# RoboticsDesignLab/jitterbug

Measured on AMD Instinct MI355X. Metric: env steps/s at N_envs=4096, move_from_origin, higher is better.
Workload: dtype f32

## Files before the change

jitterbug_amd/csrc/jb_lane.hpp:

```cpp
#pragma once
#include <cmath>
#include <cstdint>
#include <type_traits>
#if !defined(__HIPCC__)
#include <atomic>
#include <thread>
#endif

#if defined(__HIPCC__)
#include <hip/hip_runtime.h>
#define JB_HD __host__ __device__ __forceinline__
#define JB_D __device__ __forceinline__
#else
#define JB_HD inline
#define JB_D inline
#endif

namespace jb {

#if defined(__HIPCC__)
JB_D float dpp_quad_xor1(float x) {
    return __builtin_bit_cast(float, __builtin_amdgcn_update_dpp(0, __builtin_bit_cast(int, x), 0xB1, 0xF, 0xF, false));
}
JB_D float dpp_quad_xor2(float x) {
    return __builtin_bit_cast(float, __builtin_amdgcn_update_dpp(0, __builtin_bit_cast(int, x), 0x4E, 0xF, 0xF, false));
}
JB_D float quad_sum(float x) {
    x += dpp_quad_xor1(x);
    x += dpp_quad_xor2(x);
    return x;
}
JB_D unsigned quad_sum_u(unsigned x) {
    x += (unsigned)__builtin_amdgcn_update_dpp(0, (int)x, 0xB1, 0xF, 0xF, false);
    x += (unsigned)__builtin_amdgcn_update_dpp(0, (int)x, 0x4E, 0xF, 0xF, false);
    return x;
}
JB_D bool any_lane(bool m) { return __builtin_amdgcn_ballot_w64(m) != 0ull; }
JB_D unsigned xor_sum_bits(unsigned u, int off, bool sym2, bool is_float) {
    auto add = [&](unsigned a, unsigned b) { return is_float ? __builtin_bit_cast(unsigned, __builtin_bit_cast(float, a) + __builtin_bit_cast(float, b)) : a + b; };
    if (off == 32) { auto r = __builtin_amdgcn_permlane32_swap(u, u, false, false); return add(r[0], r[1]); }
    if (off == 16) { auto r = __builtin_amdgcn_permlane16_swap(u, u, false, false); return add(r[0], r[1]); }
    if (off == 8) return add(u, (unsigned)__builtin_amdgcn_update_dpp(0, (int)u, 0x128, 0xF, 0xF, false));
    if (off == 4 && sym2) return add(u, (unsigned)__builtin_amdgcn_update_dpp(0, (int)u, 0x124, 0xF, 0xF, false));
    return add(u, (unsigned)__shfl_xor((int)u, off, 64));
}
JB_D float row_transpose_sum(float v0, float v1, float v2, float v3) {
    auto f = [](unsigned u) { return __builtin_bit_cast(float, u); };
    auto b = [](float x) { return __builtin_bit_cast(unsigned, x); };
    auto r02 = __builtin_amdgcn_permlane32_swap(b(v0), b(v2), false, false);
    auto r13 = __builtin_amdgcn_permlane32_swap(b(v1), b(v3), false, false);
    float s02 = f(r02[0]) + f(r02[1]), s13 = f(r13[0]) + f(r13[1]);
    auto r = __builtin_amdgcn_permlane16_swap(b(s02), b(s13), false, false);
    return f(r[0]) + f(r[1]);
}
JB_D unsigned xor_get_bits(unsigned u, int off) {
    if (off == 32) { auto r = __builtin_amdgcn_permlane32_swap(u, u, false, false); return r[1]; }
    if (off == 16) { auto r = __builtin_amdgcn_permlane16_swap(u, u, false, false); return r[1]; }
    if (off == 8) return (unsigned)__builtin_amdgcn_update_dpp(0, (int)u, 0x128, 0xF, 0xF, false);
    return (unsigned)__shfl_xor((int)u, off, 64);
}
JB_D unsigned xor_get_any_u(unsigned u, int off) {
    if (off == 32) { auto r = __builtin_amdgcn_permlane32_swap(u, u, false, false); return r[0] ^ r[1] ^ u; }
    if (off == 16) { auto r = __builtin_amdgcn_permlane16_swap(u, u, false, false); return r[0] ^ r[1] ^ u; }
    return xor_get_bits(u, off);
}
JB_D float xor_get(float x, int off) { return __builtin_bit_cast(float, xor_get_bits(__builtin_bit_cast(unsigned, x), off)); }
JB_D unsigned xor_get_u(unsigned x, int off) { return xor_get_bits(x, off); }
template <int J> JB_D float quad_bcast(float x) { return __builtin_bit_cast(float, __builtin_amdgcn_update_dpp(0, __builtin_bit_cast(int, x), J * 0x55, 0xF, 0xF, false)); }
JB_D float xor_sum(float x, int off, bool sym2) { return __builtin_bit_cast(float, xor_sum_bits(__builtin_bit_cast(unsigned, x), off, sym2, true)); }
JB_D unsigned xor_sum_u(unsigned x, int off, bool sym2) { return xor_sum_bits(x, off, sym2, false); }
JB_D unsigned wave_bcast_u(unsigned x) { return (unsigned)__builtin_amdgcn_readfirstlane((int)x); }
JB_D void wave_sync() {
    __builtin_amdgcn_fence(__ATOMIC_RELEASE, "wavefront");
    __builtin_amdgcn_wave_barrier();
    __builtin_amdgcn_fence(__ATOMIC_ACQUIRE, "wavefront");
}
template <int K> JB_D float quad_rot(float x) {
    constexpr int ctrl = K == 1 ? 0x39 : K == 2 ? 0x4E : 0x93;
    return __builtin_bit_cast(float, __builtin_amdgcn_update_dpp(0, __builtin_bit_cast(int, x), ctrl, 0xF, 0xF, false));
}
template <int K> JB_D unsigned quad_rot_u(unsigned x) {
    constexpr int ctrl = K == 1 ? 0x39 : K == 2 ? 0x4E : 0x93;
    return (unsigned)__builtin_amdgcn_update_dpp(0, (int)x, ctrl, 0xF, 0xF, false);
}
template <int J> JB_D unsigned quad_bcast_u(unsigned x) { return (unsigned)__builtin_amdgcn_update_dpp(0, (int)x, J * 0x55, 0xF, 0xF, false); }
JB_D unsigned quad_lane_id(const float*) { return threadIdx.x & 3u; }
JB_D float ld_leg(const float* p, int stride, unsigned idx, unsigned src, unsigned me) { return p[(int)(idx * (unsigned)stride) + (int)src - (int)me]; }
JB_D void st_leg(float* p, int stride, unsigned idx, unsigned src, unsigned me, float v, bool on) { if (on) p[(int)(idx * (unsigned)stride) + (int)src - (int)me] = v; }
JB_D float quad_pick(float x, unsigned src) {
    const int xi = __builtin_bit_cast(int, x);
    const float x0 = __builtin_bit_cast(float, __builtin_amdgcn_update_dpp(0, xi, 0x00, 0xF, 0xF, false)), x1 = __builtin_bit_cast(float, __builtin_amdgcn_update_dpp(0, xi, 0x55, 0xF, 0xF, false));
    const float x2 = __builtin_bit_cast(float, __builtin_amdgcn_update_dpp(0, xi, 0xAA, 0xF, 0xF, false)), x3 = __builtin_bit_cast(float, __builtin_amdgcn_update_dpp(0, xi, 0xFF, 0xF, 0xF, false));
    const float lo = (src & 1u) ? x1 : x0, hi = (src & 1u) ? x3 : x2;
    return (src & 2u) ? hi : lo;
}
#endif

JB_HD float sel(bool m, float a, float b) { return m ? a : b; }
JB_HD double sel(bool m, double a, double b) { return m ? a : b; }
JB_HD unsigned selu(bool m, unsigned a, unsigned b) { return m ? a : b; }
JB_HD bool lt(float a, float b) { return a < b; }
JB_HD bool lt(double a, double b) { return a < b; }
JB_HD bool gt(float a, float b) { return a > b; }
JB_HD bool gt(double a, double b) { return a > b; }
JB_HD bool mand(bool a, bool b) { return a && b; }
JB_HD bool mor(bool a, bool b) { return a || b; }
JB_HD bool mnot(bool a) { return !a; }
JB_HD unsigned mbit(bool a) { return a ? 1u : 0u; }
JB_HD unsigned popc_u(unsigned a) { return (unsigned)__builtin_popcount(a); }
JB_HD unsigned xor_u(unsigned a, unsigned b) { return a ^ b; }
JB_HD bool eq_u(unsigned a, unsigned b) { return a == b; }
JB_HD bool lt_u(unsigned a, unsigned b) { return a < b; }
JB_HD unsigned or_u(unsigned a, unsigned b) { return a | b; }
JB_HD unsigned and_u(unsigned a, unsigned b) { return a & b; }
JB_HD unsigned sub_u(unsigned a, unsigned b) { return a - b; }
JB_HD unsigned shl_u(unsigned a, unsigned s) { return a << s; }
JB_HD unsigned ctz_u(unsigned a) { return a ? (unsigned)__builtin_ctz(a) : 0u; }
JB_HD unsigned clear_low_u(unsigned a) { return a & (a - 1u); }
JB_HD float utov(unsigned a, const float*) { return (float)a; }
JB_HD double utov(unsigned a, const double*) { return (double)a; }
JB_HD void flip_decode(unsigned diff0, unsigned diff1, unsigned rec0, unsigned rec1, unsigned live, unsigned& entry, bool& is_flip, bool& plus, bool& tan2, bool& on) {
    const bool w1 = diff0 == 0u;
    const unsigned diff = w1 ? diff1 : diff0, rec = w1 ? rec1 : rec0;
// ... 101 lines not shown
inline void wave_sync() { if (g_host_wave) g_host_wave->barrier(); }
template <typename T> inline Quad<T> host_exchange(const Quad<T>& x, int partner) {
    HostWave* w = g_host_wave;
    for (int i = 0; i < 4; i++) w->mbox[g_host_grp][0][i] = (double)x.v[i];
    w->barrier();
    Quad<T> r;
    for (int i = 0; i < 4; i++) r.v[i] = (T)w->mbox[partner][0][i];
    w->barrier();
    return r;
}
template <typename T> inline Quad<T> row_transpose_sum(const Quad<T>& v0, const Quad<T>& v1, const Quad<T>& v2, const Quad<T>& v3) {
    HostWave* w = g_host_wave;
    if (!w) return v0;
    const Quad<T>* v[4] = {&v0, &v1, &v2, &v3};
    for (int k = 0; k < 4; k++) for (int i = 0; i < 4; i++) w->mbox[g_host_grp][k][i] = (double)v[k]->v[i];
    w->barrier();
    Quad<T> r;
    const int g = g_host_grp;
    for (int i = 0; i < 4; i++) r.v[i] = ((T)w->mbox[0][g][i] + (T)w->mbox[2][g][i]) + ((T)w->mbox[1][g][i] + (T)w->mbox[3][g][i]);
    w->barrier();
    return r;
}
template <typename T> inline Quad<T> xor_sum(const Quad<T>& x, int off, bool) {
    if (!g_host_wave) return x;
    return x + host_exchange(x, g_host_grp ^ (off / g_host_wave->gstride));
}
inline UQuad xor_sum_u(const UQuad& x, int off, bool) {
    HostWave* w = g_host_wave;
    if (!w) return x;
    for (int i = 0; i < 4; i++) w->umbox[g_host_grp][i] = x.v[i];
    w->barrier();
    UQuad r;
    const int partner = g_host_grp ^ (off / w->gstride);
    for (int i = 0; i < 4; i++) r.v[i] = x.v[i] + w->umbox[partner][i];
    w->barrier();
    return r;
}
template <typename T> inline Quad<T> xor_get(const Quad<T>& x, int off) {
    if (!g_host_wave) return x;
    return host_exchange(x, g_host_grp ^ (off / g_host_wave->gstride));
}
inline UQuad xor_get_u(const UQuad& x, int off) {
    HostWave* w = g_host_wave;
    if (!w) return x;
    for (int i = 0; i < 4; i++) w->umbox[g_host_grp][i] = x.v[i];
    w->barrier();
    UQuad r;
    const int partner = g_host_grp ^ (off / w->gstride);
    for (int i = 0; i < 4; i++) r.v[i] = w->umbox[partner][i];
    w->barrier();
    return r;
}
inline UQuad xor_get_any_u(const UQuad& x, int off) { return xor_get_u(x, off); }
template <int J, typename T> inline Quad<T> quad_bcast(const Quad<T>& x) { return Quad<T>(x.v[J]); }
inline unsigned wave_bcast_u(unsigned x) {
    HostWave* w = g_host_wave;
    if (!w) return x;
    w->umbox[g_host_grp][0] = x;
    w->barrier();
    const unsigned r = w->umbox[0][0];
    w->barrier();
    return r;
}
inline bool any_lane(bool m) { return m; }
inline float quad_sum(float x) { return x; }
inline double quad_sum(double x) { return x; }
template <typename T> inline Quad<T> sel(const Mask4& m, const Quad<T>& a, const Quad<T>& b) { Quad<T> r; for (int i = 0; i < 4; i++) r.v[i] = m.v[i] ? a.v[i] : b.v[i]; return r; }
inline UQuad selu(const Mask4& m, const UQuad& a, const UQuad& b) { UQuad r; for (int i = 0; i < 4; i++) r.v[i] = m.v[i] ? a.v[i] : b.v[i]; return r; }
template <typename T> inline Mask4 lt(const Quad<T>& a, const Quad<T>& b) { Mask4 r; for (int i = 0; i < 4; i++) r.v[i] = a.v[i] < b.v[i]; return r; }
template <typename T> inline Mask4 gt(const Quad<T>& a, const Quad<T>& b) { Mask4 r; for (int i = 0; i < 4; i++) r.v[i] = a.v[i] > b.v[i]; return r; }
inline Mask4 mand(const Mask4& a, const Mask4& b) { Mask4 r; for (int i = 0; i < 4; i++) r.v[i] = a.v[i] && b.v[i]; return r; }
inline Mask4 mor(const Mask4& a, const Mask4& b) { Mask4 r; for (int i = 0; i < 4; i++) r.v[i] = a.v[i] || b.v[i]; return r; }
inline Mask4 mnot(const Mask4& a) { Mask4 r; for (int i = 0; i < 4; i++) r.v[i] = !a.v[i]; return r; }
inline UQuad mbit(const Mask4& a) { UQuad r; for (int i = 0; i < 4; i++) r.v[i] = a.v[i] ? 1u : 0u; return r; }
inline UQuad popc_u(const UQuad& a) { UQuad r; for (int i = 0; i < 4; i++) r.v[i] = (uint32_t)__builtin_popcount(a.v[i]); return r; }
inline UQuad xor_u(const UQuad& a, const UQuad& b) { UQuad r; for (int i = 0; i < 4; i++) r.v[i] = a.v[i] ^ b.v[i]; return r; }
inline Mask4 lt_u(const UQuad& a, uint32_t b) { Mask4 r; for (int i = 0; i < 4; i++) r.v[i] = a.v[i] < b; return r; }
inline UQuad or_u(const UQuad& a, const UQuad& b) { UQuad r; for (int i = 0; i < 4; i++) r.v[i] = a.v[i] | b.v[i]; return r; }
inline UQuad and_u(const UQuad& a, const UQuad& b) { UQuad r; for (int i = 0; i < 4; i++) r.v[i] = a.v[i] & b.v[i]; return r; }
inline UQuad and_u(const UQuad& a, uint32_t b) { UQuad r; for (int i = 0; i < 4; i++) r.v[i] = a.v[i] & b; return r; }
inline UQuad sub_u(const UQuad& a, const UQuad& b) { UQuad r; for (int i = 0; i < 4; i++) r.v[i] = a.v[i] - b.v[i]; return r; }
inline UQuad shl_u(const UQuad& a, const UQuad& s) { UQuad r; for (int i = 0; i < 4; i++) r.v[i] = a.v[i] << s.v[i]; return r; }
inline UQuad ctz_u(const UQuad& a) { UQuad r; for (int i = 0; i < 4; i++) r.v[i] = a.v[i] ? (uint32_t)__builtin_ctz(a.v[i]) : 0u; return r; }
inline UQuad clear_low_u(const UQuad& a) { UQuad r; for (int i = 0; i < 4; i++) r.v[i] = a.v[i] & (a.v[i] - 1u); return r; }
inline Mask4 lt_u(const UQuad& a, const UQuad& b) { Mask4 r; for (int i = 0; i < 4; i++) r.v[i] = a.v[i] < b.v[i]; return r; }
inline Mask4 eq_u(const UQuad& a, uint32_t b) { Mask4 r; for (int i = 0; i < 4; i++) r.v[i] = a.v[i] == b; return r; }
template <typename T> inline Quad<T> utov(const UQuad& a, const Quad<T>*) { Quad<T> r; for (int i = 0; i < 4; i++) r.v[i] = (T)a.v[i]; return r; }
template <int K, typename T> inline Quad<T> quad_rot(const Quad<T>& x) { Quad<T> r; for (int i = 0; i < 4; i++) r.v[i] = x.v[(i + K) & 3]; return r; }
template <int K> inline UQuad quad_rot_u(const UQuad& x) { UQuad r; for (int i = 0; i < 4; i++) r.v[i] = x.v[(i + K) & 3]; return r; }
template <int J> inline UQuad quad_bcast_u(const UQuad& x) { return UQuad{{x.v[J], x.v[J], x.v[J], x.v[J]}}; }
template <typename T> inline UQuad quad_lane_id(const Quad<T>*) { return UQuad{{0u, 1u, 2u, 3u}}; }
template <typename T> inline void st_leg(Quad<T>* p, int stride, const UQuad& idx, const UQuad& src, const UQuad&, const Quad<T>& v, const Mask4& on) { for (int i = 0; i < 4; i++) if (on.v[i]) p[idx.v[i] * stride].v[src.v[i]] = v.v[i]; }
template <typename T> inline Quad<T> quad_pick(const Quad<T>& x, const UQuad& src) { Quad<T> r; for (int i = 0; i < 4; i++) r.v[i] = x.v[src.v[i]]; return r; }
template <typename T> inline Quad<T> ld_leg(const Quad<T>* p, int stride, const UQuad& idx, const UQuad& src, const UQuad&) { Quad<T> r; for (int i = 0; i < 4; i++) r.v[i] = p[idx.v[i] * stride].v[src.v[i]]; return r; }
inline Mask4 eq_u(const UQuad& a, const UQuad& b) { Mask4 r; for (int i = 0; i < 4; i++) r.v[i] = a.v[i] == b.v[i]; return r; }
inline void flip_decode(const UQuad& diff0, const UQuad& diff1, const UQuad& rec0, const UQuad& rec1, unsigned live, UQuad& entry, Mask4& is_flip, Mask4& plus, Mask4& tan2, Mask4& on) {
    for (int i = 0; i < 4; i++) flip_decode(diff0.v[i], diff1.v[i], rec0.v[i], rec1.v[i], live, entry.v[i], is_flip.v[i], plus.v[i], tan2.v[i], on.v[i]);
}
template <typename T> inline Quad<T> ld_gather(const Quad<T>* p, int stride, const UQuad& idx) { Quad<T> r; for (int i = 0; i < 4; i++) r.v[i] = p[idx.v[i] * stride].v[i]; return r; }
inline Mask4 neq_u(const UQuad& a, const UQuad& b) { Mask4 r; for (int i = 0; i < 4; i++) r.v[i] = a.v[i] != b.v[i]; return r; }
inline UQuad operator*(const UQuad& a, uint32_t b) { UQuad r; for (int i = 0; i < 4; i++) r.v[i] = a.v[i] * b; return r; }
inline UQuad operator+(const UQuad& a, const UQuad& b) { UQuad r; for (int i = 0; i < 4; i++) r.v[i] = a.v[i] + b.v[i]; return r; }
inline UQuad operator+(const UQuad& a, uint32_t b) { UQuad r; for (int i = 0; i < 4; i++) r.v[i] = a.v[i] + b; return r; }
#define JB_QUN(name, fn) template <typename T> inline Quad<T> name(const Quad<T>& a) { Quad<T> r; for (int i = 0; i < 4; i++) r.v[i] = fn(a.v[i]); return r; }
template <typename T> inline Quad<T> vmul_rn(const Quad<T>& a, const Quad<T>& b) { Quad<T> r; for (int i = 0; i < 4; i++) r.v[i] = vmul_rn(a.v[i], b.v[i]); return r; }
template <typename T> inline Quad<T> vadd_rn(const Quad<T>& a, const Quad<T>& b) { Quad<T> r; for (int i = 0; i < 4; i++) r.v[i] = vadd_rn(a.v[i], b.v[i]); return r; }
// ... 55 lines not shown
```

jitterbug_amd/csrc/jb_sim.hpp:

```cpp
#pragma once
#include <type_traits>
#if !defined(__HIPCC__)
#include <cstdio>
#endif

#include "jb_lane.hpp"

#if defined(__HIPCC__) && defined(__HIP_DEVICE_COMPILE__)
#define JB_SCHED_FENCE() __builtin_amdgcn_sched_barrier(0)
#define JB_ASM_MARK(txt) asm volatile("; " txt)
#else
#define JB_ASM_MARK(txt) ((void)0)
#define JB_NO_DEVICE_PROF 1
#define JB_SCHED_FENCE() ((void)0)
#endif

#if defined(JB_WAVE_STATS) && !defined(JB_NO_DEVICE_PROF)
#define JB_PROF_T0() unsigned long long _pt = __builtin_amdgcn_s_memtime()
#define JB_PROF_ADD(o, i) do { unsigned long long _n = __builtin_amdgcn_s_memtime(); if ((o).prof) (o).prof[i] += _n - _pt; _pt = _n; } while (0)
#else
#define JB_PROF_T0() ((void)0)
#define JB_PROF_ADD(o, i) ((void)0)
#endif

// ... 242 lines not shown
    V fail;
#ifdef JB_WAVE_STATS
    V st_fast, st_checks;
    V st_xtra, st_sweeps, st_contact, st_slots;
#endif
};

constexpr int NSLOT = 30, SLOT_THREAD = 28, SLOT_MASS = 29;
constexpr int ROW_F = 13;
constexpr int ROW_K = JB_ROW_K;
enum SC : int {
    SC_DD = 0 ,
    SC_Y = 24 ,
    SC_ST = SC_Y + 9 ,
    SC_OWN = SC_ST + 6 ,
    SC_ROWS = SC_OWN + 1 ,
    SC_VAR = SC_ROWS + ROW_K * ROW_F ,
    SC_RED = SC_VAR ,
    SC_OVC = SC_RED + 56 ,
    SC_PD = SC_OVC + 4 * (NSLOT - ROW_K) ,
    SC_PD2 = SC_PD + 12 ,
    SC_ZERO = SC_PD2 + 9 ,
    SC_COUNT = SC_ZERO + 56,
    SC_SYS = SC_VAR , SC_FAC = SC_SYS + 41 , SC_LSTATE = SC_FAC + 43 ,
    SC_COUNT_LEAN = SC_LSTATE + 36,
    SC_CX_LEAN = SC_COUNT_LEAN , SC_PD_LEAN = SC_CX_LEAN + 2 , SC_COUNT_LEAN_PAIR = SC_PD_LEAN + 12
};
template <typename V> struct LaneScratch {
    V* p;
    int stride;
    int grp, ngrp, gstride;
    V* ovc;
    int ovc_stride;
    int pd;
    int pd2;
    bool aux_lane = false;
    bool red_lds;
    JB_HD V ld(int i) const { return p[i * stride]; }
    JB_HD void st(int i, const V& v) const { p[i * stride] = v; }
    JB_HD V ldv(const typename lane_traits<V>::uint& i) const { return ld_gather(p, stride, i); }
    JB_HD Vec3<V> ld3(int i) const { return v3<V>(ld(i), ld(i + 1), ld(i + 2)); }
    JB_HD void st3(int i, const Vec3<V>& v) const { st(i, v.x); st(i + 1, v.y); st(i + 2, v.z); }
};
template <typename V> JB_HD V group_sum(const LaneScratch<V>& sc, V x) {
    if (sc.ngrp == 4) { x = xor_sum(x, 2 * sc.gstride, false); x = xor_sum(x, sc.gstride, true); }
    else if (sc.ngrp == 2) x = xor_sum(x, sc.gstride, false);
    return x;
}
template <typename V> JB_HD typename lane_traits<V>::uint group_sum_u(const LaneScratch<V>& sc, typename lane_traits<V>::uint x) {
    if (sc.ngrp == 4) { x = xor_sum_u(x, 2 * sc.gstride, false); x = xor_sum_u(x, sc.gstride, true); }
    else if (sc.ngrp == 2) x = xor_sum_u(x, sc.gstride, false);
    return x;
}
template <typename V> JB_HD int ls_mailbox(const LaneScratch<V>& sc) { return sc.red_lds ? (int)SC_RED : (int)SC_FAC; }
JB_HD constexpr int tri(int i, int j) { return i >= j ? i * (i + 1) / 2 + j : j * (j + 1) / 2 + i; }

JB_HD constexpr int s6base(int j) { return j == 0 ? 0 : j == 1 ? 3 : j == 2 ? 6 : j == 3 ? 8 : j == 4 ? 10 : 11; }
JB_HD constexpr int s6p(int ip, int j) { return s6base(j) + ip - j / 2; }
template <typename V> struct Sym6P { Pk2<V> p[12]; };
template <typename V> JB_HD V pk_half(const Pk2<V>& w, int h) { return h ? pk_hi(w) : pk_lo(w); }
template <typename V> JB_HD Pk2<V> pk_with(const Pk2<V>& w, int h, const V& x) { return h ? Pk2<V>(pk_lo(w), x) : Pk2<V>(x, pk_hi(w)); }
template <typename V> JB_HD V s6get(const Sym6P<V>& S, int i, int j) { return i >= j ? pk_half(S.p[s6p(i >> 1, j)], i & 1) : pk_half(S.p[s6p(j >> 1, i)], j & 1); }
template <typename V> JB_HD void s6set(Sym6P<V>& S, int i, int j, const V& x) { S.p[s6p(i >> 1, j)] = pk_with(S.p[s6p(i >> 1, j)], i & 1, x); }
template <typename V> JB_HD V v6get(const Pk2<V> (&v)[3], int i) { return pk_half(v[i >> 1], i & 1); }
template <typename V> JB_HD void v6set(Pk2<V> (&v)[3], int i, const V& x) { v[i >> 1] = pk_with(v[i >> 1], i & 1, x); }
template <typename V> JB_HD V b6get(const Pk2<V> (&B)[3][2], int i, int c) { return pk_half(B[i >> 1][c], i & 1); }
template <typename V, typename MKT> JB_HD Pk2<V> selw(const MKT& k, const Pk2<V>& a, const Pk2<V>& b) { return Pk2<V>(sel(k, pk_lo(a), pk_lo(b)), sel(k, pk_hi(a), pk_hi(b))); }
template <typename V> JB_HD Pk2<V> qsum2(const Pk2<V>& a) { return Pk2<V>(quad_sum(pk_lo(a)), quad_sum(pk_hi(a))); }
template <typename V> JB_HD Pk2<V> qsum_hi(const Pk2<V>& a) { return Pk2<V>(pk_lo(a), quad_sum(pk_hi(a))); }
JB_HD constexpr bool s6_junk_lo(int ip, int j) { return 2 * ip < j; }

template <typename V> struct NewtonAcc {
    Sym6P<V> A;
    Pk2<V> B[3][2];
    V C11, C12, C22;
    V X;
    Pk2<V> Bm[3]; V Cm;
    Pk2<V> rr[3]; V rl[2], rm;
    typename lane_traits<V>::uint bw0, bw1;
    typename lane_traits<V>::uint xh;
    V ls_g, ls_h, ls_a;
};
template <typename V> struct LineDir { V dr[6], dl[2], dm, alpha; };
template <typename V> JB_HD void acc_clear(NewtonAcc<V>& acc) {
    using W = Pk2<V>;
#pragma unroll
    for (int i = 0; i < 12; i++) acc.A.p[i] = W(0);
#pragma unroll
    for (int i = 0; i < 3; i++) { acc.B[i][0] = W(0); acc.B[i][1] = W(0); acc.Bm[i] = W(0); acc.rr[i] = W(0); }
    acc.C11 = V(0); acc.C12 = V(0); acc.C22 = V(0); acc.Cm = V(0); acc.X = V(0);
    acc.rl[0] = V(0); acc.rl[1] = V(0); acc.rm = V(0);
    acc.bw0 = zero_u<V>(); acc.bw1 = zero_u<V>(); acc.xh = zero_u<V>();
}

template <typename V> JB_HD void acc_pack(const NewtonAcc<V>& a, V* v) {
#pragma unroll
    for (int i = 0; i < 6; i++)
#pragma unroll
        for (int j = 0; j <= i; j++) v[tri(i, j)] = s6get(a.A, i, j);
#pragma unroll
    for (int i = 0; i < 6; i++) { v[21 + 2 * i] = b6get(a.B, i, 0); v[22 + 2 * i] = b6get(a.B, i, 1); v[36 + i] = v6get(a.Bm, i); v[43 + i] = v6get(a.rr, i); }
    v[33] = a.C11; v[34] = a.C12; v[35] = a.C22; v[42] = a.Cm; v[49] = a.rl[0]; v[50] = a.rl[1]; v[51] = a.rm;
}
template <typename V> JB_HD void acc_unpack(const V* v, NewtonAcc<V>& a) {
    using W = Pk2<V>;
#pragma unroll
    for (int j = 0; j < 6; j++)
#pragma unroll
        for (int ip = j / 2; ip < 3; ip++) a.A.p[s6p(ip, j)] = W(v[tri(2 * ip, j)], v[tri(2 * ip + 1, j)]);
#pragma unroll
    for (int ip = 0; ip < 3; ip++) {
        a.B[ip][0] = W(v[21 + 4 * ip], v[23 + 4 * ip]); a.B[ip][1] = W(v[22 + 4 * ip], v[24 + 4 * ip]);
        a.Bm[ip] = W(v[36 + 2 * ip], v[37 + 2 * ip]); a.rr[ip] = W(v[43 + 2 * ip], v[44 + 2 * ip]);
    }
    a.C11 = v[33]; a.C12 = v[34]; a.C22 = v[35]; a.Cm = v[42]; a.rl[0] = v[49]; a.rl[1] = v[50]; a.rm = v[51];
}

template <typename V> struct StarSys {
    Sym6P<V> A;
    Pk2<V> B[3][2];
    V C[3];
    Pk2<V> Bm[3]; V Cm;
    Pk2<V> tr[3]; V tl[2], tm;
};

template <typename V> struct StarFactor {
    Sym6P<V> S;
    Pk2<V> B[3][2];
    V i11, i12, i22;
    Pk2<V> bm[3]; V icm;
    V cx0, cx1;
};
template <typename V, bool WITH_ACC = true, bool PAIR = false>
JB_HD void star_factor(const StarSys<V>& M, const NewtonAcc<V>& acc, const V& hb1, const V& hb2, StarFactor<V>& F) {
    using W = Pk2<V>;
#pragma unroll
    for (int ip = 0; ip < 3; ip++) {
        F.B[ip][0] = WITH_ACC ? M.B[ip][0] + acc.B[ip][0] : M.B[ip][0];
        F.B[ip][1] = WITH_ACC ? M.B[ip][1] + acc.B[ip][1] : M.B[ip][1];
    }
    V C11 = M.C[0] + hb1, C12 = M.C[1], C22 = M.C[2] + hb2;
    if (WITH_ACC) { C11 = M.C[0] + acc.C11 + hb1; C12 = M.C[1] + acc.C12; C22 = M.C[2] + acc.C22 + hb2; }
    V idet = vrcp(C11 * C22 - C12 * C12);
    F.i11 = C22 * idet; F.i12 = -C12 * idet; F.i22 = C11 * idet;
    Sym6P<V>& S = F.S;
    W g[3][2];
#pragma unroll
    for (int ip = 0; ip < 3; ip++) {
        g[ip][0] = F.B[ip][0] * W(F.i11) + F.B[ip][1] * W(F.i12);
        g[ip][1] = F.B[ip][0] * W(F.i12) + F.B[ip][1] * W(F.i22);
    }
#pragma unroll
    for (int j = 0; j < 6; j++) {
        const V bj0 = b6get(F.B, j, 0), bj1 = b6get(F.B, j, 1);
#pragma unroll
        for (int ip = j / 2; ip < 3; ip++) {
            const W leg = g[ip][0] * W(bj0) + g[ip][1] * W(bj1);
            const int k = s6p(ip, j);
            if (WITH_ACC) { const W t = acc.A.p[k] - leg; S.p[k] = (s6_junk_lo(ip, j) ? qsum_hi(t) : qsum2(t)) + M.A.p[k]; }
            else S.p[k] = M.A.p[k] - (s6_junk_lo(ip, j) ? qsum_hi(leg) : qsum2(leg));
        }
    }
    V cm = M.Cm;
#pragma unroll
    for (int ip = 0; ip < 3; ip++) F.bm[ip] = M.Bm[ip];
    if (WITH_ACC) {
#pragma unroll
        for (int ip = 0; ip < 3; ip++) F.bm[ip] = F.bm[ip] + qsum2(acc.Bm[ip]);
// ... 621 lines not shown
    for (int ip = 0; ip < 3; ip++) yr[ip] = Pk2<V>(sc.ld(SC_Y + 2 * ip), sc.ld(SC_Y + 2 * ip + 1));
    yl[0] = sc.ld(SC_Y + 6); yl[1] = sc.ld(SC_Y + 7); ym = sc.ld(SC_Y + 8);
    const int g = plan.grouped ? sc.grp : 0;
    unsigned rest_mine = plan.mine;
    int rest_rounds = plan.rounds;
    if (sp.on) {
        using U = typename lane_traits<V>::uint;
        const U me = quad_lane_id((const V*)nullptr);
#pragma unroll 1
        for (int r = 0;; r++) {
            const SpreadItem<V> it = r == 0 ? sp.item0 : spread_assign<V>(sp.own, sp.mg, r);
            const U below = sub_u(shl_u(zero_u<V>() + 1u, it.slot), zero_u<V>() + 1u);
            const U e0 = popc_u(and_u(below, zero_u<V>() + plan.live)) * (unsigned)ROW_F + (unsigned)SC_ROWS;
            RowVals<V> rv;
            rv.x = v3<V>(ld_leg(sc.p, sc.stride, e0, it.src, me), ld_leg(sc.p, sc.stride, e0 + 1u, it.src, me), ld_leg(sc.p, sc.stride, e0 + 2u, it.src, me));
            rv.D = ld_leg(sc.p, sc.stride, e0 + 3u, it.src, me);
#pragma unroll
            for (int k = 0; k < 3; k++) {
                rv.jsh[k] = ld_leg(sc.p, sc.stride, e0 + (unsigned)(4 + k), it.src, me); rv.j7[k] = ld_leg(sc.p, sc.stride, e0 + (unsigned)(7 + k), it.src, me);
                rv.ah[k] = ld_leg(sc.p, sc.stride, e0 + (unsigned)(10 + k), it.src, me);
            }
            V yls[2];
            yls[0] = ld_leg(sc.p, sc.stride, zero_u<V>() + (unsigned)(SC_Y + 6), it.src, me); yls[1] = ld_leg(sc.p, sc.stride, zero_u<V>() + (unsigned)(SC_Y + 7), it.src, me);
            if (LS && mode == 3) {
                V dls[2];
                dls[0] = ld_leg(sc.p, sc.stride, zero_u<V>() + (unsigned)(box + 6), it.src, me); dls[1] = ld_leg(sc.p, sc.stride, zero_u<V>() + (unsigned)(box + 7), it.src, me);
                contact_apply_leg<V, LS>(rv, dk, mu, it, 3, yr, yls, acc, &ldir, dls);
            } else contact_apply_leg<V, LS>(rv, dk, mu, it, mode, yr, yls, acc);
            spread_rounds = r + 1;
            if (!any_lane(it.more)) break;
        }
        rest_mine = sp.rest_mine; rest_rounds = sp.rest_rounds;
    }
#pragma unroll 1
    for (int r = 0; r < rest_rounds; r++) {
        const int mine = r < __builtin_popcount(rest_mine) ? nth_set_bit(rest_mine, r) : -1;
        const bool lane_on = mine >= 0 && !(g1z && !plan.grouped);
        const int slot = lane_on ? mine : __builtin_ctz(sp.on ? (plan.live & ~sp.slots) : plan.live);
        const int rank = plan_rank(plan, slot);
        RowVals<V> rv;
        if (rank < ROW_K) row_load<V>(sc, rank, rv);
        else {
            const int c0 = 4 * (rank - ROW_K) * sc.ovc_stride;
            row_values<V, PAIR>(m, sc, xtra, slot, v3<V>(sc.ovc[c0], sc.ovc[c0 + sc.ovc_stride], sc.ovc[c0 + 2 * sc.ovc_stride]), sc.ovc[c0 + 3 * sc.ovc_stride], rv);
        }
        contact_apply<V, PAIR, LS>(rv, dk, mu, slot, lane_on, mode, yr, yl, ym, acc, (LS && mode == 3) ? &ldir : nullptr);
    }
    if (LS && mode == 3) {
        acc.ls_g = quad_sum(acc.ls_g); acc.ls_h = quad_sum(acc.ls_h); acc.ls_a = quad_sum(acc.ls_a);
        if (plan.grouped) { acc.ls_g = group_sum(sc, acc.ls_g); acc.ls_h = group_sum(sc, acc.ls_h); acc.ls_a = group_sum(sc, acc.ls_a); }
        return spread_rounds + 8 * rest_rounds;
    }
    if (plan.grouped) {
        acc.bw0 = group_sum_u<V>(sc, acc.bw0); acc.bw1 = group_sum_u<V>(sc, acc.bw1); acc.xh = group_sum_u<V>(sc, acc.xh);
        if (mode == 0 && sc.ngrp == 4 && sc.gstride == 16 && sc.red_lds) {
            constexpr int NQ4 = PAIR ? 14 : 13;
            V v[56];
            acc_pack(acc, v);
            if (PAIR) { v[52] = acc.X; v[53] = V(0); v[54] = V(0); v[55] = V(0); }
            static_assert(4 * NQ4 <= 56, "reduction buffer");
#pragma unroll
            for (int k = 0; k < NQ4; k++) sc.st(SC_RED + 4 * k + sc.grp, row_transpose_sum(v[4 * k], v[4 * k + 1], v[4 * k + 2], v[4 * k + 3]));
            wave_sync();
            if (sc.grp == 0 || g1z) {
                const int src = g1z ? SC_ZERO : SC_RED;
#pragma unroll
                for (int i = 0; i < (PAIR ? 53 : 52); i++) v[i] = sc.ld(src + i);
                acc_unpack(v, acc);
                if (PAIR) acc.X = v[52];
            }
        } else if (mode == 0) {
            V v[52];
            acc_pack(acc, v);
#pragma unroll
            for (int i = 0; i < 52; i++) v[i] = group_sum(sc, v[i]);
            acc_unpack(v, acc);
            if (PAIR) acc.X = group_sum(sc, acc.X);
            if (g1z) acc_clear(acc);
        }
    }
    return spread_rounds + 8 * rest_rounds;
}

template <typename V> struct CylContacts {
    Vec3<V> x[4];
    V dist[4];
    typename lane_traits<V>::mask on[4];
};
template <typename V>
JB_HD void cylinder_floor(const Vec3<V>& c, const Vec3<V>& ax_in, const Vec3<V>& xa, const V& rad, const V& half, const Vec3<V>& nb, const V& pz, const V& pz_lo,
                          const typename lane_traits<V>::mask& enabled, CylContacts<V>& out) {
    V prj = dot(ax_in, nb);
    auto flip = gt(prj, V(0));
    Vec3<V> ax = v3<V>(sel(flip, -ax_in.x, ax_in.x), sel(flip, -ax_in.y, ax_in.y), sel(flip, -ax_in.z, ax_in.z));
    prj = sel(flip, -prj, prj);
    V dist0 = (pz + dot(c, nb)) + pz_lo;
    Vec3<V> vec = ax * prj - nb;
    V len2 = dot(vec, vec);
    auto degenerate = lt(len2, V(1e-20));
    V scl = rad * vrsqrt(vmax(len2, V(1e-30)));
    vec = v3<V>(sel(degenerate, xa.x * rad, vec.x * scl), sel(degenerate, xa.y * rad, vec.y * scl), sel(degenerate, xa.z * rad, vec.z * scl));
    V prjvec = dot(vec, nb);
    Vec3<V> axh = ax * half;
    V prjaxis = prj * half;
    V d1 = dist0 + prjaxis + prjvec;
    auto on1 = mand(enabled, lt(d1, V(0)));
    if (!any_lane(on1)) {
#pragma unroll
        for (int k = 0; k < 4; k++) { out.dist[k] = V(1); out.on[k] = on1; out.x[k] = c; }
        return;
    }
    out.dist[0] = d1; out.on[0] = on1;
    out.x[0] = c + vec + axh - nb * (d1 * V(0.5));
    V d2 = dist0 - prjaxis + prjvec;
    out.dist[1] = d2; out.on[1] = mand(on1, lt(d2, V(0)));
    out.x[1] = c + vec - axh - nb * (d2 * V(0.5));
    V d3 = dist0 + prjaxis - V(0.5) * prjvec;
    auto on3 = mand(on1, lt(d3, V(0)));
    Vec3<V> v1 = cross(vec, axh);
    v1 = v1 * (rad * V(0.8660254037844386) * vrsqrt(vmax(dot(v1, v1), V(1e-30))));
    Vec3<V> base = c + axh - vec * V(0.5) - nb * (d3 * V(0.5));
    out.dist[2] = d3; out.on[2] = on3; out.x[2] = base + v1;
    out.dist[3] = d3; out.on[3] = on3; out.x[3] = base - v1;
}


template <typename V, typename MKT>
JB_HD unsigned cand_store(const LaneScratch<V>& sc, unsigned live_before, int slot, const Vec3<V>& x, const V& dist, const MKT& on, typename lane_traits<V>::uint* own = nullptr) {
// ... 910 lines not shown
                    pon = mand(near_pair, lt(pdist, V(0)));
                }
                if (any_lane(pon)) {
                    const Vec3<V> wy = v3<V>(R.m[3], R.m[4], R.m[5]);
                    const V ny = dot(pn, wy);
                    const Vec3<V> ys = sel_v3(lt(vabs(ny), V(0.5)), wy, nb);
                    Vec3<V> t1 = ys - pn * dot(pn, ys);
                    t1 = t1 * vrsqrt(vmax(dot(t1, t1), V(1e-30)));
                    sc.st3(sc.pd, pn); sc.st3(sc.pd + 3, t1); sc.st3(sc.pd + 6, cross(pn, t1));
                }
                sc.st(sc.pd + 11, sel(near_pair, V(1), V(0)));
                live_slots |= cand_store(sc, live_slots, SLOT_MASS, ppos, pdist, pon);
                any_con = mor(any_con, pon);
            }
            any_contact = any_lane(any_con);
            env_con = neq_u(quad_sum_u(mbit(any_con)), zero_u<V>());
            if (o.aux) {
                const U ec = xor_get_any_u(mbit(env_con), axoff);
                if (axl) env_con = neq_u(ec, zero_u<V>());
            }
            if (any_contact && !axl) sc.st(SC_OWN, utov(own, (const V*)nullptr));
            if (any_contact && !axl) {
#pragma unroll
                for (int k = 0; k < 3; k++) {
                    Vec3<V> d = (k == 0) ? nb : (k == 1) ? v3<V>(R.m[3], R.m[4], R.m[5]) : v3<V>(-R.m[0], -R.m[1], -R.m[2]);
                    sc.st3(SC_DD + 3 * k, d);
                    sc.st(SC_DD + 21 + k, dot(d, u));
                }
                sc.st3(SC_DD + 9, e1); sc.st3(SC_DD + 12, a1); sc.st3(SC_DD + 15, e2); sc.st3(SC_DD + 18, a2);
            }
        }
        JB_SCHED_FENCE();

        const W mw = W(m1, m2);
        const Vec3<W> hw = ccw * mw;
        const Sym3<W> Jo = about_origin(Iw, mw, ccw);
        const Sym3<V> J2 = hi(Jo);
        const Sym3<V> J12 = lo(Jo) + J2;
        const Vec3<V> h2 = hi(hw), h12 = lo(hw) + h2;
        const V m12 = m1 + m2;
        const Vec3<W> sw = cross(aw, ew);
        const Vec3<W> hcw = pk(h12, h2);
        const Vec3<W> fw = sw * W(m12, m2) + cross(ew, hcw), nw = mul(pk(J12, J2), ew) + cross(hcw, sw);
        const Vec3<V> fS = lo(fw), fK = hi(fw), nS = lo(nw), nK = hi(nw);
        sys.B[0][0] = W(nS.x, nS.y); sys.B[1][0] = W(nS.z, fS.x); sys.B[2][0] = W(fS.y, fS.z);
        sys.B[0][1] = W(nK.x, nK.y); sys.B[1][1] = W(nK.z, fK.x); sys.B[2][1] = W(fK.y, fK.z);
        {
            const W cd = dot(ew, nw) + dot(sw, fw);
            sys.C[0] = pk_lo(cd); sys.C[2] = pk_hi(cd);
            sys.C[1] = dot(e1, nK) + dot(lo(sw), fK);
        }
        const Vec3<V> h12q = qsum(h12);
        const Sym3<V> J12q = qsum(J12);
        Vec3<V> ht;
        Sym3<V> Jt;
        if (o.aux) {
            ht = v3<V>(xor_get(h12q.x, axoff), xor_get(h12q.y, axoff), xor_get(h12q.z, axoff)) + h12q;
            Sym3<V> Jx;
            Jx.xx = xor_get(J12q.xx, axoff); Jx.yy = xor_get(J12q.yy, axoff); Jx.zz = xor_get(J12q.zz, axoff);
            Jx.xy = xor_get(J12q.xy, axoff); Jx.xz = xor_get(J12q.xz, axoff); Jx.yz = xor_get(J12q.yz, axoff);
            Jt = Jx + J12q;
#pragma unroll
            for (int ip = 0; ip < 3; ip++) sys.Bm[ip] = W(xor_get(quad_bcast<0>(pk_lo(sys.B[ip][0])), axoff), xor_get(quad_bcast<0>(pk_hi(sys.B[ip][0])), axoff));
            sys.Cm = xor_get(quad_bcast<0>(sys.C[0]), axoff);
        } else {
            Vec3<V> sM = cross(am, em);
            Vec3<V> hm = cm * mm;
            Sym3<V> Jm = about_origin(Im, mm, cm);
            Vec3<V> fM = sM * mm + cross(em, hm), nM = mul(Jm, em) + cross(hm, sM);
            sys.Bm[0] = W(nM.x, nM.y); sys.Bm[1] = W(nM.z, fM.x); sys.Bm[2] = W(fM.y, fM.z);
            sys.Cm = dot(em, nM) + dot(sM, fM);
            ht = c0 * m0 + hm + h12q;
            Jt = about_origin(I0, m0, c0) + Jm + J12q;
        }
        root_block<V>(Jt, ht, m.c[LM_MTOT], sys.A);
        JB_SCHED_FENCE();

        {
            const V w_2 = dot(w, w);
            auto accel_at = [&](const Vec3<V>& x) { return AO + wxwx(w, w_2, x); };
            const Vec3<V> Aa1 = accel_at(a1);
            const Vec3<V> w1 = w + e1 * s.thd1, w2 = w1 + e2 * s.thd2;
            const Vec3<W> www = pk(w1, w2);
            const Vec3<W> dal = cross(pk(w, w1), ew) * W(s.thd1, s.thd2);
            const Vec3<V> al1 = lo(dal), al2 = al1 + hi(dal);
            const Vec3<W> alw = pk(al1, al2);
            const Vec3<W> rw = ccw - aw;
            const W w2w = dot(www, www);
            const Vec3<V> r12 = a2 - a1;
            const Vec3<V> Aa2 = Aa1 + cross(al1, r12) + wxwx(w1, pk_lo(w2w), r12);
            const Vec3<W> Fw = (pk(Aa1, Aa2) + cross(alw, rw) + wxwx(www, w2w, rw)) * mw;
            const Vec3<W> Nw = mul(Iw, alw) + cross(www, mul(Iw, www));
            const Vec3<W> tw = Nw + cross(rw, Fw);
            const Vec3<V> F2 = hi(Fw);
            V cK = dot(e2, hi(tw));
            V cS = dot(e1, lo(tw) + hi(Nw) + cross(cc2 - a1, F2));
            Vec3<V> legF = lo(Fw) + F2;
            const Vec3<W> Now = Nw + cross(ccw, Fw);
            Vec3<V> legN = lo(Now) + hi(Now);
            const Vec3<V> legFq = qsum(legF), legNq = qsum(legN);
            Vec3<V> bl, ba;
            V cM;
            if (o.aux) {
                bl = v3<V>(xor_get(legFq.x, axoff), xor_get(legFq.y, axoff), xor_get(legFq.z, axoff)) + legFq;
                ba = v3<V>(xor_get(legNq.x, axoff), xor_get(legNq.y, axoff), xor_get(legNq.z, axoff)) + legNq;
                cM = xor_get(quad_bcast<0>(cS), axoff);
            } else {
                Vec3<V> F0 = accel_at(c0) * m0;
                Vec3<V> N0 = cross(w, mul(I0, w));
                Vec3<V> wm = w + em * s.phid;
                Vec3<V> alm = cross(w, em) * s.phid;
                Vec3<V> rm = cm - am;
                Vec3<V> Fm = (accel_at(am) + cross(alm, rm) + wxwx(wm, dot(wm, wm), rm)) * mm;
                Vec3<V> Nm = mul(Im, alm) + cross(wm, mul(Im, wm));
                cM = dot(em, Nm + cross(rm, Fm));
                bl = F0 + Fm + legFq;
                ba = N0 + cross(c0, F0) + Nm + cross(cm, Fm) + legNq;
            }
            sys.tr[0] = W(-ba.x, -ba.y); sys.tr[1] = W(-ba.z, -bl.x); sys.tr[2] = W(-bl.y, -bl.z);
            sys.tl[0] = -cS - m.c[LM_K1] * s.th1 - m.c[LM_B1] * s.thd1;
            sys.tl[1] = -cK - m.c[LM_K2] * s.th2 - m.c[LM_B2] * s.thd2;
            V uc = vmin(vmax(ctrl, m.c[LM_CTRL_LO]), m.c[LM_CTRL_HI]);
            V gear = m.c[LM_GEAR];
            V len = gear * (s.phi + s.turns * V(6.283185307179586));
            V force = m.c[LM_GAIN] * uc + m.c[LM_BIAS] + m.c[LM_BIAS + 1] * len + m.c[LM_BIAS + 2] * gear * s.phid;
            sys.tm = -cM + gear * force;
        }
    }
    JB_SCHED_FENCE();
    if (o.lean && is_main) sys_store(sc, sys);

    JB_PROF_ADD(o, 0);
    any_contact = wave_bcast_u(any_contact ? 1u : 0u) != 0u;
    live_slots = wave_bcast_u(live_slots);
    wave_sync();
    const SlotPlan plan = make_slot_plan(sc, live_slots);
    const SpreadPlan<V> spl = make_spread_plan<V>(sc, plan, o.spread != 0 && any_contact);

    Vec3<V> dk[3];
    if (any_contact) {
#pragma unroll
        for (int k = 0; k < 3; k++) dk[k] = sc.ld3(SC_DD + 3 * k);
        contact_rows_build_all<V, PAIR>(m, sc, xtra, plan, spl);
        JB_PROF_ADD(o, 5);
    }
    Pk2<V> yrp[3];
    V yl[2], ym;
    MK capped = lt(V(1), V(0));
    bool redone = newton_phase<V, PAIR, false>(m, sc, s, o, xtra, plan, spl, Rw, sys, dk, any_contact, env_con, yrp, yl, ym, capped);
#ifdef JB_NO_RESOLVE
    redone = false;
#endif
    if (__builtin_expect(redone, false)) {
        JB_ASM_MARK("jb-cold-solve-begin");
        const U cf = group_sum_u<V>(sc, mbit(capped));
        Pk2<V> zr[3];
        V zl[2], zm;
        MK capped2 = lt(V(1), V(0));
        (void)newton_phase<V, PAIR, true>(m, sc, s, o, xtra, plan, spl, Rw, sys, dk, any_contact, env_con, zr, zl, zm, capped2);
// ... 119 lines not shown
```

Baseline: 7.111 million.

## Reuse permlane swap spare operands and repack Newton accumulator reductions

Cross-half lane exchanges now carry a spare register through successive permlane32/16 swaps, so each swap delivers a useful value instead of discarding one output. The Newton accumulator packing is reordered into paired slots, so the LDS transpose-reduction uses a three-input variant for the final row and skips summing mirrored symmetric entries, which are copied instead. All groups now load unconditionally from either the reduction or zero region. The intent is fewer cross-lane instructions and less redundant reduction work; the risk is subtle lane-data correctness bugs from the spare-value chaining.

```diff
diff --git a/jitterbug_amd/csrc/jb_lane.hpp b/jitterbug_amd/csrc/jb_lane.hpp
--- a/jitterbug_amd/csrc/jb_lane.hpp
+++ b/jitterbug_amd/csrc/jb_lane.hpp
@@ -66,9 +66,38 @@
 }
 JB_D float xor_get(float x, int off) { return __builtin_bit_cast(float, xor_get_bits(__builtin_bit_cast(unsigned, x), off)); }
 JB_D unsigned xor_get_u(unsigned x, int off) { return xor_get_bits(x, off); }
+JB_D float xor_sum_lower(float x, int off, unsigned& spare) {
+    auto f = [](unsigned u) { return __builtin_bit_cast(float, u); };
+    const unsigned u = __builtin_bit_cast(unsigned, x);
+    if (off == 32) { auto r = __builtin_amdgcn_permlane32_swap(u, spare, false, false); const float s = f(r[1]) + f(r[0]); spare = r[1]; return s; }
+    if (off == 16) { auto r = __builtin_amdgcn_permlane16_swap(u, spare, false, false); const float s = f(r[1]) + f(r[0]); spare = r[1]; return s; }
+    return f(xor_get_bits(u, off)) + x;
+}
+JB_D float xor_fetch(float x, int off, unsigned& spare) {
+    const unsigned u = __builtin_bit_cast(unsigned, x);
+    if (off == 32) { auto r = __builtin_amdgcn_permlane32_swap(u, spare, false, false); spare = r[0]; return __builtin_bit_cast(float, r[1]); }
+    if (off == 16) { auto r = __builtin_amdgcn_permlane16_swap(u, spare, false, false); spare = r[0]; return __builtin_bit_cast(float, r[1]); }
+    return __builtin_bit_cast(float, xor_get_bits(u, off));
+}
 template <int J> JB_D float quad_bcast(float x) { return __builtin_bit_cast(float, __builtin_amdgcn_update_dpp(0, __builtin_bit_cast(int, x), J * 0x55, 0xF, 0xF, false)); }
 JB_D float xor_sum(float x, int off, bool sym2) { return __builtin_bit_cast(float, xor_sum_bits(__builtin_bit_cast(unsigned, x), off, sym2, true)); }
 JB_D unsigned xor_sum_u(unsigned x, int off, bool sym2) { return xor_sum_bits(x, off, sym2, false); }
+JB_D unsigned xor_sum_lower_u(unsigned x, int off, bool sym2, unsigned& spare) {
+    if (off == 32) { auto r = __builtin_amdgcn_permlane32_swap(x, spare, false, false); const unsigned s = r[0] + r[1]; spare = r[1]; return s; }
+    if (off == 16) { auto r = __builtin_amdgcn_permlane16_swap(x, spare, false, false); const unsigned s = r[0] + r[1]; spare = r[1]; return s; }
+    return xor_sum_u(x, off, sym2);
+}
+template <typename V> JB_D unsigned swap_spare_u() { return __builtin_nondeterministic_value(0u); }
+JB_D float row_transpose_sum3(float v0, float v1, float v2) {
+    auto f = [](unsigned u) { return __builtin_bit_cast(float, u); };
+    auto b = [](float x) { return __builtin_bit_cast(unsigned, x); };
+    auto r02 = __builtin_amdgcn_permlane32_swap(b(v0), b(v2), false, false);
+    const float s02 = f(r02[0]) + f(r02[1]);
+    auto r13 = __builtin_amdgcn_permlane32_swap(b(v1), r02[1], false, false);
+    const float s13 = f(r13[0]) + f(r13[1]);
+    auto r = __builtin_amdgcn_permlane16_swap(b(s02), b(s13), false, false);
+    return f(r[0]) + f(r[1]);
+}
 JB_D unsigned wave_bcast_u(unsigned x) { return (unsigned)__builtin_amdgcn_readfirstlane((int)x); }
 JB_D void wave_sync() {
     __builtin_amdgcn_fence(__ATOMIC_RELEASE, "wavefront");
@@ -276,6 +305,11 @@
     return r;
 }
 inline UQuad xor_get_any_u(const UQuad& x, int off) { return xor_get_u(x, off); }
+template <typename T> inline Quad<T> xor_sum_lower(const Quad<T>& x, int off, UQuad&) { const Quad<T> r = xor_get(x, off); return r + x; }
+template <typename T> inline Quad<T> xor_fetch(const Quad<T>& x, int off, UQuad&) { return xor_get(x, off); }
+inline UQuad xor_sum_lower_u(const UQuad& x, int off, bool sym2, UQuad&) { return xor_sum_u(x, off, sym2); }
+template <typename V> inline UQuad swap_spare_u() { return UQuad{{0u, 0u, 0u, 0u}}; }
+template <typename T> inline Quad<T> row_transpose_sum3(const Quad<T>& v0, const Quad<T>& v1, const Quad<T>& v2) { return row_transpose_sum(v0, v1, v2, v2); }
 template <int J, typename T> inline Quad<T> quad_bcast(const Quad<T>& x) { return Quad<T>(x.v[J]); }
 inline unsigned wave_bcast_u(unsigned x) {
     HostWave* w = g_host_wave;
diff --git a/jitterbug_amd/csrc/jb_sim.hpp b/jitterbug_amd/csrc/jb_sim.hpp
--- a/jitterbug_amd/csrc/jb_sim.hpp
+++ b/jitterbug_amd/csrc/jb_sim.hpp
@@ -318,6 +318,16 @@
     else if (sc.ngrp == 2) x = xor_sum_u(x, sc.gstride, false);
     return x;
 }
+template <typename V> JB_HD void group_sum_main_u(const LaneScratch<V>& sc, typename lane_traits<V>::uint& a, typename lane_traits<V>::uint& b, typename lane_traits<V>::uint& c) {
+    typename lane_traits<V>::uint spare = swap_spare_u<V>();
+    if (sc.ngrp == 4) {
+        a = xor_sum_lower_u(a, 2 * sc.gstride, false, spare); a = xor_sum_lower_u(a, sc.gstride, true, spare);
+        b = xor_sum_lower_u(b, 2 * sc.gstride, false, spare); b = xor_sum_lower_u(b, sc.gstride, true, spare);
+        c = xor_sum_lower_u(c, 2 * sc.gstride, false, spare); c = xor_sum_lower_u(c, sc.gstride, true, spare);
+    } else if (sc.ngrp == 2) {
+        a = xor_sum_lower_u(a, sc.gstride, false, spare); b = xor_sum_lower_u(b, sc.gstride, false, spare); c = xor_sum_lower_u(c, sc.gstride, false, spare);
+    }
+}
 template <typename V> JB_HD int ls_mailbox(const LaneScratch<V>& sc) { return sc.red_lds ? (int)SC_RED : (int)SC_FAC; }
 JB_HD constexpr int tri(int i, int j) { return i >= j ? i * (i + 1) / 2 + j : j * (j + 1) / 2 + i; }
 
@@ -359,27 +369,36 @@
     acc.bw0 = zero_u<V>(); acc.bw1 = zero_u<V>(); acc.xh = zero_u<V>();
 }
 
+constexpr int ACC_PAIRS = 24, ACC_NV = 2 * ACC_PAIRS + 7, ACC_X = ACC_NV;
+JB_HD constexpr int acc_pair_A(int q) { return q; }
+JB_HD constexpr int acc_pair_B(int ip, int c) { return 12 + 2 * ip + c; }
+JB_HD constexpr int acc_pair_Bm(int ip) { return 18 + ip; }
+JB_HD constexpr int acc_pair_rr(int ip) { return 21 + ip; }
+JB_HD constexpr int acc_mirror_of(int e) {
+    return e == 2 * s6p(0, 1) ? 2 * s6p(0, 0) + 1 : e == 2 * s6p(1, 3) ? 2 * s6p(1, 2) + 1 : e == 2 * s6p(2, 5) ? 2 * s6p(2, 4) + 1 : -1;
+}
 template <typename V> JB_HD void acc_pack(const NewtonAcc<V>& a, V* v) {
 #pragma unroll
-    for (int i = 0; i < 6; i++)
-#pragma unroll
-        for (int j = 0; j <= i; j++) v[tri(i, j)] = s6get(a.A, i, j);
-#pragma unroll
-    for (int i = 0; i < 6; i++) { v[21 + 2 * i] = b6get(a.B, i, 0); v[22 + 2 * i] = b6get(a.B, i, 1); v[36 + i] = v6get(a.Bm, i); v[43 + i] = v6get(a.rr, i); }
-    v[33] = a.C11; v[34] = a.C12; v[35] = a.C22; v[42] = a.Cm; v[49] = a.rl[0]; v[50] = a.rl[1]; v[51] = a.rm;
+    for (int q = 0; q < 12; q++) { v[2 * acc_pair_A(q)] = pk_lo(a.A.p[q]); v[2 * acc_pair_A(q) + 1] = pk_hi(a.A.p[q]); }
+#pragma unroll
+    for (int ip = 0; ip < 3; ip++) {
+#pragma unroll
+        for (int c = 0; c < 2; c++) { v[2 * acc_pair_B(ip, c)] = pk_lo(a.B[ip][c]); v[2 * acc_pair_B(ip, c) + 1] = pk_hi(a.B[ip][c]); }
+        v[2 * acc_pair_Bm(ip)] = pk_lo(a.Bm[ip]); v[2 * acc_pair_Bm(ip) + 1] = pk_hi(a.Bm[ip]);
+        v[2 * acc_pair_rr(ip)] = pk_lo(a.rr[ip]); v[2 * acc_pair_rr(ip) + 1] = pk_hi(a.rr[ip]);
+    }
+    v[48] = a.C11; v[49] = a.C12; v[50] = a.C22; v[51] = a.Cm; v[52] = a.rl[0]; v[53] = a.rl[1]; v[54] = a.rm;
 }
 template <typename V> JB_HD void acc_unpack(const V* v, NewtonAcc<V>& a) {
     using W = Pk2<V>;
 #pragma unroll
-    for (int j = 0; j < 6; j++)
-#pragma unroll
-        for (int ip = j / 2; ip < 3; ip++) a.A.p[s6p(ip, j)] = W(v[tri(2 * ip, j)], v[tri(2 * ip + 1, j)]);
+    for (int q = 0; q < 12; q++) a.A.p[q] = W(v[2 * acc_pair_A(q)], v[2 * acc_pair_A(q) + 1]);
 #pragma unroll
     for (int ip = 0; ip < 3; ip++) {
-        a.B[ip][0] = W(v[21 + 4 * ip], v[23 + 4 * ip]); a.B[ip][1] = W(v[22 + 4 * ip], v[24 + 4 * ip]);
-        a.Bm[ip] = W(v[36 + 2 * ip], v[37 + 2 * ip]); a.rr[ip] = W(v[43 + 2 * ip], v[44 + 2 * ip]);
-    }
-    a.C11 = v[33]; a.C12 = v[34]; a.C22 = v[35]; a.Cm = v[42]; a.rl[0] = v[49]; a.rl[1] = v[50]; a.rm = v[51];
+        a.B[ip][0] = W(v[2 * acc_pair_B(ip, 0)], v[2 * acc_pair_B(ip, 0) + 1]); a.B[ip][1] = W(v[2 * acc_pair_B(ip, 1)], v[2 * acc_pair_B(ip, 1) + 1]);
+        a.Bm[ip] = W(v[2 * acc_pair_Bm(ip)], v[2 * acc_pair_Bm(ip) + 1]); a.rr[ip] = W(v[2 * acc_pair_rr(ip)], v[2 * acc_pair_rr(ip) + 1]);
+    }
+    a.C11 = v[48]; a.C12 = v[49]; a.C22 = v[50]; a.Cm = v[51]; a.rl[0] = v[52]; a.rl[1] = v[53]; a.rm = v[54];
 }
 
 template <typename V> struct StarSys {
@@ -1107,28 +1126,29 @@
         return spread_rounds + 8 * rest_rounds;
     }
     if (plan.grouped) {
-        acc.bw0 = group_sum_u<V>(sc, acc.bw0); acc.bw1 = group_sum_u<V>(sc, acc.bw1); acc.xh = group_sum_u<V>(sc, acc.xh);
-        if (mode == 0 && sc.ngrp == 4 && sc.gstride == 16 && sc.red_lds) {
-            constexpr int NQ4 = PAIR ? 14 : 13;
-            V v[56];
+        group_sum_main_u<V>(sc, acc.bw0, acc.bw1, acc.xh);
+        if (mode == 0 && !LS && sc.ngrp == 4 && sc.gstride == 16 && sc.red_lds) {
+            constexpr int NQ4 = 14;
+            V v[4 * NQ4];
+            static_assert(ACC_X < 4 * NQ4 && 4 * NQ4 <= 56, "reduction buffer");
             acc_pack(acc, v);
-            if (PAIR) { v[52] = acc.X; v[53] = V(0); v[54] = V(0); v[55] = V(0); }
-            static_assert(4 * NQ4 <= 56, "reduction buffer");
-#pragma unroll
-            for (int k = 0; k < NQ4; k++) sc.st(SC_RED + 4 * k + sc.grp, row_transpose_sum(v[4 * k], v[4 * k + 1], v[4 * k + 2], v[4 * k + 3]));
+            if (PAIR) v[ACC_X] = acc.X;
+#pragma unroll
+            for (int k = 0; k < NQ4 - 1; k++) sc.st(SC_RED + 4 * k + sc.grp, row_transpose_sum(v[4 * k], v[4 * k + 1], v[4 * k + 2], v[4 * k + 3]));
+            sc.st(SC_RED + 4 * (NQ4 - 1) + sc.grp, PAIR ? row_transpose_sum(v[ACC_X - 3], v[ACC_X - 2], v[ACC_X - 1], v[ACC_X]) : row_transpose_sum3(v[ACC_X - 3], v[ACC_X - 2], v[ACC_X - 1]));
             wave_sync();
-            if (sc.grp == 0 || g1z) {
-                const int src = g1z ? SC_ZERO : SC_RED;
-#pragma unroll
-                for (int i = 0; i < (PAIR ? 53 : 52); i++) v[i] = sc.ld(src + i);
-                acc_unpack(v, acc);
-                if (PAIR) acc.X = v[52];
-            }
+            const int src = sc.grp == 0 ? SC_RED : SC_ZERO;
+#pragma unroll
+            for (int i = 0; i < (PAIR ? ACC_NV + 1 : ACC_NV); i++) v[i] = sc.ld(src + i);
+            acc_unpack(v, acc);
+            if (PAIR) acc.X = v[ACC_X];
         } else if (mode == 0) {
-            V v[52];
+            V v[ACC_NV];
             acc_pack(acc, v);
 #pragma unroll
-            for (int i = 0; i < 52; i++) v[i] = group_sum(sc, v[i]);
+            for (int i = 0; i < ACC_NV; i++) if (acc_mirror_of(i) < 0) v[i] = group_sum(sc, v[i]);
+#pragma unroll
+            for (int i = 0; i < ACC_NV; i++) if (acc_mirror_of(i) >= 0) v[i] = v[acc_mirror_of(i)];
             acc_unpack(v, acc);
             if (PAIR) acc.X = group_sum(sc, acc.X);
             if (g1z) acc_clear(acc);
@@ -2145,17 +2165,19 @@
         }
         const Vec3<V> h12q = qsum(h12);
         const Sym3<V> J12q = qsum(J12);
+        U spare = swap_spare_u<V>();
         Vec3<V> ht;
         Sym3<V> Jt;
         if (o.aux) {
-            ht = v3<V>(xor_get(h12q.x, axoff), xor_get(h12q.y, axoff), xor_get(h12q.z, axoff)) + h12q;
-            Sym3<V> Jx;
-            Jx.xx = xor_get(J12q.xx, axoff); Jx.yy = xor_get(J12q.yy, axoff); Jx.zz = xor_get(J12q.zz, axoff);
-            Jx.xy = xor_get(J12q.xy, axoff); Jx.xz = xor_get(J12q.xz, axoff); Jx.yz = xor_get(J12q.yz, axoff);
-            Jt = Jx + J12q;
-#pragma unroll
-            for (int ip = 0; ip < 3; ip++) sys.Bm[ip] = W(xor_get(quad_bcast<0>(pk_lo(sys.B[ip][0])), axoff), xor_get(quad_bcast<0>(pk_hi(sys.B[ip][0])), axoff));
-            sys.Cm = xor_get(quad_bcast<0>(sys.C[0]), axoff);
+            ht = v3<V>(xor_sum_lower(h12q.x, axoff, spare), xor_sum_lower(h12q.y, axoff, spare), xor_sum_lower(h12q.z, axoff, spare));
+            Jt.xx = xor_sum_lower(J12q.xx, axoff, spare); Jt.yy = xor_sum_lower(J12q.yy, axoff, spare); Jt.zz = xor_sum_lower(J12q.zz, axoff, spare);
+            Jt.xy = xor_sum_lower(J12q.xy, axoff, spare); Jt.xz = xor_sum_lower(J12q.xz, axoff, spare); Jt.yz = xor_sum_lower(J12q.yz, axoff, spare);
+#pragma unroll
+            for (int ip = 0; ip < 3; ip++) {
+                const V blo = xor_fetch(quad_bcast<0>(pk_lo(sys.B[ip][0])), axoff, spare), bhi = xor_fetch(quad_bcast<0>(pk_hi(sys.B[ip][0])), axoff, spare);
+                sys.Bm[ip] = W(blo, bhi);
+            }
+            sys.Cm = xor_fetch(quad_bcast<0>(sys.C[0]), axoff, spare);
         } else {
             Vec3<V> sM = cross(am, em);
             Vec3<V> hm = cm * mm;
@@ -2195,9 +2217,9 @@
             Vec3<V> bl, ba;
             V cM;
             if (o.aux) {
-                bl = v3<V>(xor_get(legFq.x, axoff), xor_get(legFq.y, axoff), xor_get(legFq.z, axoff)) + legFq;
-                ba = v3<V>(xor_get(legNq.x, axoff), xor_get(legNq.y, axoff), xor_get(legNq.z, axoff)) + legNq;
-                cM = xor_get(quad_bcast<0>(cS), axoff);
+                bl = v3<V>(xor_sum_lower(legFq.x, axoff, spare), xor_sum_lower(legFq.y, axoff, spare), xor_sum_lower(legFq.z, axoff, spare));
+                ba = v3<V>(xor_sum_lower(legNq.x, axoff, spare), xor_sum_lower(legNq.y, axoff, spare), xor_sum_lower(legNq.z, axoff, spare));
+                cM = xor_fetch(quad_bcast<0>(cS), axoff, spare);
             } else {
                 Vec3<V> F0 = accel_at(c0) * m0;
                 Vec3<V> N0 = cross(w, mul(I0, w));
```

After: 3.725 million. -47.6%, worse.
